# amisr/volumetricinterp

Measured on AMD Instinct MI355X. Metric: fit+eval timesteps/sec, higher is better.
Workload: dtype f64

## Files before the change

### volumetricinterp_amd/csrc/vi_jacobi.hip

```cpp
#include "vi_common.h"
#include "vi_solver.h"

#include <cstdlib>
#include <cstring>

#ifdef VI_STAMPS
__device__ unsigned long long g_jacobi_stamps[16];
#define VI_STAMP(k)                                                                          \
    do {                                                                                     \
        const unsigned long long t_ = __builtin_readcyclecounter();                          \
        if (blockIdx.x == 0 && (threadIdx.x == 0 || threadIdx.x == blockDim.x - 64))         \
            g_jacobi_stamps[(threadIdx.x == 0 ? 0 : 8) + (k)] += t_ - stamp_t;               \
        stamp_t = __builtin_readcyclecounter();                                              \
    } while (0)
#else
#define VI_STAMP(k)
#endif

#ifdef VI_ROTHIST
__device__ unsigned long long g_rot_hist[32][2];
#define VI_ROT_COUNT(sweep, r0, r1, r2, r3)                                                                              \
    atomicAdd(&g_rot_hist[(sweep) < 31 ? (sweep) : 31][0],                                                               \
              (unsigned long long)(((r0).y != 0.0) + ((r1).y != 0.0) + ((r2).y != 0.0) + ((r3).y != 0.0)))
#define VI_ROT_SWEEP(sweep)                                                                                               \
    do { if (threadIdx.x == 0) atomicAdd(&g_rot_hist[(sweep) < 31 ? (sweep) : 31][1], 1ull); } while (0)
#endif

#include "vi_jacobi_device.h"
#include "vi_jacobi_v2_device.h"
#include <cstdlib>
#include <cstring>

namespace {

template <int IT>
__global__ __launch_bounds__(IT == 1 ? 768 : 512) void k_jacobi_solve(
    int N, const double* __restrict__ X, const double* __restrict__ scl, const double* __restrict__ y,
    const int* __restrict__ rec, double rcond, double abs_floor, double* __restrict__ C, int* __restrict__ rank,
    double2* __restrict__ rotlog, int64_t log_stride, int max_sweeps, int* __restrict__ sweeps_out,
    double* __restrict__ lam_out, int lam_raw, int* __restrict__ nround_out, unsigned long long* __restrict__ round_acc,
    double conv_tol)
{
    extern __shared__ __align__(16) unsigned char lds_raw[];
    const int64_t sys = blockIdx.x;
    jacobi_system<IT>(lds_raw, N, X + sys * (int64_t)N * N, scl ? scl[sys] : 1.0, y + (int64_t)(rec ? rec[sys] : sys) * N, rcond,
                      abs_floor, C + sys * N, rank ? rank + sys : nullptr, rotlog + sys * log_stride, max_sweeps,
                      sweeps_out ? sweeps_out + sys : nullptr, lam_out ? lam_out + sys * N : nullptr, lam_raw,
                      nround_out ? nround_out + sys : nullptr, round_acc, conv_tol);
}

__global__ __launch_bounds__(768) void k_jacobi_solve_v2(
    int N, const double* __restrict__ X, const double* __restrict__ scl, const double* __restrict__ y,
    const int* __restrict__ rec, double rcond, double abs_floor, double* __restrict__ C, int* __restrict__ rank,
    double2* __restrict__ rotlog, int64_t log_stride, int max_sweeps, int* __restrict__ sweeps_out,
    double* __restrict__ lam_out, int lam_raw, int* __restrict__ nround_out, unsigned long long* __restrict__ round_acc,
    double conv_tol)
{
    extern __shared__ __align__(16) unsigned char lds_raw[];
    const int64_t sys = blockIdx.x;
    jacobi_system_v2(lds_raw, N, X + sys * (int64_t)N * N, scl ? scl[sys] : 1.0, y + (int64_t)(rec ? rec[sys] : sys) * N, rcond,
                     abs_floor, C + sys * N, rank ? rank + sys : nullptr, rotlog + sys * log_stride, max_sweeps,
                     sweeps_out ? sweeps_out + sys : nullptr, lam_out ? lam_out + sys * N : nullptr, lam_raw,
                     nround_out ? nround_out + sys : nullptr, round_acc, conv_tol);
}

template <int CPW>
__global__ __launch_bounds__(64) void k_jacobi_vectors_wave(int N, const double2* __restrict__ rotlog, int64_t log_stride,
                                                            const int* __restrict__ nround_in, double* __restrict__ Vout)
{
    const int64_t sys = blockIdx.y;
    jacobi_vector_strip<CPW>(N, rotlog + sys * log_stride, nround_in[sys], blockIdx.x * CPW, threadIdx.x,
                             Vout + sys * (int64_t)N * N);
}

}

#ifdef VI_STAMPS
extern "C" int vi_debug_jacobi_stamps(double* out, int reset)
{
    unsigned long long h[16];
    if (hipMemcpyFromSymbol(h, HIP_SYMBOL(g_jacobi_stamps), sizeof(h)) != hipSuccess) return -1;
    for (int i = 0; i < 16; ++i) out[i] = (double)h[i];
    if (reset) {
        memset(h, 0, sizeof(h));
        if (hipMemcpyToSymbol(HIP_SYMBOL(g_jacobi_stamps), h, sizeof(h)) != hipSuccess) return -1;
    }
    return 0;
}
#endif

#ifdef VI_ROTHIST
extern "C" int vi_debug_rot_hist(double* out, int reset)
{
    unsigned long long h[32][2];
    if (hipMemcpyFromSymbol(h, HIP_SYMBOL(g_rot_hist), sizeof(h)) != hipSuccess) return -1;
    for (int i = 0; i < 32; ++i) { out[2 * i] = (double)h[i][0]; out[2 * i + 1] = (double)h[i][1]; }
    if (reset) {
        memset(h, 0, sizeof(h));
        if (hipMemcpyToSymbol(HIP_SYMBOL(g_rot_hist), h, sizeof(h)) != hipSuccess) return -1;
    }
    return 0;
}
#endif

namespace {

int jacobi_nsb(int N)
{
    const int M = ((N + 3) & ~3) / 4;
    return M * (M - 1) / 2;
}
void jacobi_geometry(int N, int& threads, int& it)
{
    const int nsb = jacobi_nsb(N);
    if (nsb <= 768) {
        it = 1;
        threads = ((nsb + 63) / 64) * 64;
        if (threads < 64) threads = 64;
    } else {
        threads = 512;
        it = (nsb + 511) / 512;
    }
}

}

bool vi_jacobi_use_v2(int N)
{
    static const bool v1 = vi_env_is("VINTERP_K3", "v1");
    if (v1) return false;
    int threads, it;
    jacobi_geometry(N, threads, it);
    const int M = ((N + 3) & ~3) / 4;
    static const int minm = [] { const int v = vi_env_int("VINTERP_K3_MINM", 24); return v < 3 ? 3 : v; }();
    return it == 1 && M >= minm && M <= 64 && threads + 64 <= 768;
}

size_t vi_jacobi_lds_bytes(int N)
{
    const int Np = (N + 3) & ~3, M = Np / 4;
    const int nt = Np * (Np + 1) / 2;
    size_t b = (size_t)(nt + 2 * Np) * 8 + (size_t)4 * M * 16 + 16 * 8;
    if (vi_jacobi_use_v2(N)) b += (size_t)4 * M * 16 + (size_t)4 * M * 8 + 16 + (size_t)14 * M * 4;
    return (b + 15) & ~(size_t)15;
}

bool vi_jacobi_supported(int N)
{
    int threads, it;
    jacobi_geometry(N, threads, it);
    return N >= 8 && vi_jacobi_lds_bytes(N) <= 159 * 1024 && it <= 3 && ((N + 3) / 4) <= 64;
}

static int64_t jacobi_log_stride(int N, int max_sweeps)
{
    const int Np = (N + 3) & ~3, m = Np / 2, M = Np / 4;
    return (int64_t)max_sweeps * m * 4 * M;
}
size_t vi_jacobi_log_bytes(int N, int max_sweeps) { return (size_t)jacobi_log_stride(N, max_sweeps) * sizeof(double2); }

template <int IT>
static int launch_jacobi(vi_ctx* c, int threads, int64_t B, int N, const double* d_X, const double* d_scl, const double* d_y,
                         const int* d_rec, double rcond, double* d_C, int* d_rank, void* d_log, int max_sweeps,
                         int* d_sweeps, double* d_lam, int lam_raw, int* d_nround, double abs_floor, int64_t log_stride_in,
                         double conv_tol)
{
    const size_t shm = vi_jacobi_lds_bytes(N);
    VI_HIP(hipFuncSetAttribute((const void*)k_jacobi_solve<IT>, hipFuncAttributeMaxDynamicSharedMemorySize, (int)shm));
    const int64_t log_stride = log_stride_in > 0 ? log_stride_in : jacobi_log_stride(N, max_sweeps);
    const int slot = (int)(c->solve_launches % vi_ctx::NSOLVE_EV);
    if (c->solve_timing) VI_HIP(hipEventRecord(c->evs[slot][0], c->stream));
    hipLaunchKernelGGL(k_jacobi_solve<IT>, dim3((unsigned)B), dim3(threads), shm, c->stream, N, d_X, d_scl, d_y, d_rec,
                       rcond, abs_floor, d_C, d_rank, (double2*)d_log, log_stride, max_sweeps, d_sweeps, d_lam, lam_raw, d_nround,
                       c->solve_timing ? c->d_rounds : nullptr, conv_tol);
    VI_HIP(hipGetLastError());
    if (c->solve_timing) {
        VI_HIP(hipEventRecord(c->evs[slot][1], c->stream));
        c->solve_launches += 1;
        c->solve_systems += B;
    }
    return VI_OK;
}

int vi_jacobi_solve(vi_ctx* c, int64_t B, int N, const double* d_X, const double* d_scl, const double* d_y,
                    const int* d_rec, double rcond, double* d_C, int* d_rank, void* d_log, int max_sweeps,
                    int* d_sweeps, double* d_lam, int lam_raw, int* d_nround, double abs_floor, int64_t log_stride, double conv_tol)
{
    int threads, it;
    jacobi_geometry(N, threads, it);
    if (vi_jacobi_use_v2(N)) {
        const size_t shm = vi_jacobi_lds_bytes(N);
        VI_HIP(hipFuncSetAttribute((const void*)k_jacobi_solve_v2, hipFuncAttributeMaxDynamicSharedMemorySize, (int)shm));
        const int64_t ls = log_stride > 0 ? log_stride : jacobi_log_stride(N, max_sweeps);
        const int slot = (int)(c->solve_launches % vi_ctx::NSOLVE_EV);
        if (c->solve_timing) VI_HIP(hipEventRecord(c->evs[slot][0], c->stream));
        hipLaunchKernelGGL(k_jacobi_solve_v2, dim3((unsigned)B), dim3(threads + 64), shm, c->stream, N, d_X, d_scl, d_y, d_rec, rcond,
                           abs_floor, d_C, d_rank, (double2*)d_log, ls, max_sweeps, d_sweeps, d_lam, lam_raw, d_nround,
                           c->solve_timing ? c->d_rounds : nullptr, conv_tol);
        VI_HIP(hipGetLastError());
        if (c->solve_timing) {
            VI_HIP(hipEventRecord(c->evs[slot][1], c->stream));
            c->solve_launches += 1;
            c->solve_systems += B;
        }
        return VI_OK;
    }
#define VI_J(IT) return launch_jacobi<IT>(c, threads, B, N, d_X, d_scl, d_y, d_rec, rcond, d_C, d_rank, d_log, max_sweeps, d_sweeps, d_lam, lam_raw, d_nround, abs_floor, log_stride, conv_tol)
    if (it <= 1) VI_J(1);
    if (it <= 2) VI_J(2);
    VI_J(3);
#undef VI_J
}

bool vi_jacobi_vectors_supported(int N) { return vi_jacobi_supported(N); }

int vi_jacobi_vectors(vi_ctx* c, int64_t B, int N, const void* d_log, int max_sweeps, const int* d_nround, double* d_V,
                      int64_t log_stride_in)
{
    const int64_t log_stride = log_stride_in > 0 ? log_stride_in : jacobi_log_stride(N, max_sweeps);
    const int64_t cols = B * N, target = (int64_t)8 * c->n_cu;
#define VI_VEC(CPW)                                                                                                           \
    hipLaunchKernelGGL(k_jacobi_vectors_wave<CPW>, dim3((unsigned)((N + CPW - 1) / CPW), (unsigned)B), dim3(64), 0, c->stream, \
                       N, (const double2*)d_log, log_stride, d_nround, d_V)
    if (cols <= target) VI_VEC(1);
    else if (cols <= 2 * target) VI_VEC(2);
    else if (cols <= 4 * target) VI_VEC(4);
    else VI_VEC(8);
#undef VI_VEC
    VI_HIP(hipGetLastError());
    return VI_OK;
}
```

### volumetricinterp_amd/csrc/vi_jacobi_v2_device.h

```cpp
#pragma once
#include "vi_jacobi_device.h"

namespace {

__device__ __forceinline__ void lds_signal(int* w, int n)
{
    asm volatile("s_waitcnt lgkmcnt(0)" ::: "memory");
    __hip_atomic_fetch_add(w, n, __ATOMIC_RELAXED, __HIP_MEMORY_SCOPE_WORKGROUP);
}
template <bool SLEEP = true>
__device__ __forceinline__ void lds_wait(int* w, int target, int& bad)
{
    const int tgt = __builtin_amdgcn_readfirstlane(target);
    int spins = 0;
#pragma nounroll
    for (;;) {
        const int v = __builtin_amdgcn_readfirstlane(__hip_atomic_load(w, __ATOMIC_RELAXED, __HIP_MEMORY_SCOPE_WORKGROUP));
        if (v >= tgt) break;
        if (++spins > (1 << 22)) { bad = 1; break; }
        if (SLEEP) __builtin_amdgcn_s_sleep(1);
    }
    asm volatile("" ::: "memory");
}

__device__ __forceinline__ void jacobi_system_v2(
    unsigned char* lds_raw, int N, const double* __restrict__ Xs, double sc, const double* __restrict__ ys, double rcond,
    double abs_floor, double* __restrict__ Cs, int* __restrict__ rank_s, double2* __restrict__ logp, int max_sweeps,
    int* __restrict__ sweeps_s, double* __restrict__ lam_s, int lam_raw, int* __restrict__ nround_s,
    unsigned long long* __restrict__ round_acc, double conv_tol = 0.0)
{
    const int NT = blockDim.x;
    const int Np = (N + 3) & ~3;
    const int m = Np >> 1;
    const int M = Np >> 2;
    const int nsb = (M * (M - 1)) >> 1;
    const int ntri = 16 * nsb + 10 * M;
    const int dg = 16 * nsb;
    double* A = reinterpret_cast<double*>(lds_raw);
    double* yv = A + ntri;
    double2* cs0 = reinterpret_cast<double2*>(yv + 2 * Np);
    double* nd = reinterpret_cast<double*>(cs0 + 8 * M);
    double* mb = nd + 16;
    int* sync = reinterpret_cast<int*>(mb + 4 * M);
    int* dtab = sync + 4;

    const int tid = threadIdx.x;
    const int nw = NT >> 6;
    const bool setup = tid < 64;

    int ka = 0, kb = 1, ksrc = 0, dst[16];
    bool live = false;
    int serves = -1, q0 = 0;
    {
        int* otab = reinterpret_cast<int*>(A);
        int* wcnt = otab + NT;
        const int lane = tid & 63, wv = tid >> 6;
        const int kn = tid - 64;
        bool isd = false;
        int sv = 0;
        if (!setup && kn < nsb) {
            int bb = (int)((1.0f + sqrtf(1.0f + 8.0f * (float)kn)) * 0.5f);
            while ((bb * (bb - 1)) / 2 > kn) --bb;
            while (((bb + 1) * bb) / 2 <= kn) ++bb;
            const int aa = kn - (bb * (bb - 1)) / 2;
            if (aa == 0 && bb == 1) { isd = true; sv = 0; }
            else if (aa == 0 && bb == 2) { isd = true; sv = 1; }
            else if (aa == M - 2 && bb == M - 1) { isd = true; sv = M - 1; }
            else if (aa >= 1 && bb == aa + 2) { isd = true; sv = aa + 1; }
        }
        const bool plain = !setup && kn < nsb && !isd;
        const unsigned long long mn = __ballot(plain);
        if (lane == 0) wcnt[wv] = __popcll(mn);
        __syncthreads();
        int before = 0;
        for (int w = 0; w < wv; ++w) before += wcnt[w];
        const unsigned long long below = lane ? (~0ull >> (64 - lane)) : 0ull;
        if (isd) otab[sv] = kn;
        if (plain) otab[M + before + __popcll(mn & below)] = kn;
        __syncthreads();
        if (!setup && kn < nsb) ksrc = otab[kn];
        __syncthreads();
    }
    if (!setup) {
        const int ko = tid - 64;
        live = ko < nsb;
        const int k = live ? ksrc : 0;
        int b = (int)((1.0f + sqrtf(1.0f + 8.0f * (float)k)) * 0.5f);
        while ((b * (b - 1)) / 2 > k) --b;
        while (((b + 1) * b) / 2 <= k) ++b;
        const int a = k - (b * (b - 1)) / 2;
        ka = live ? a : 0;
        kb = live ? b : 1;
        ksrc = k;
#pragma unroll
        for (int r = 0; r < 4; ++r)
#pragma unroll
            for (int c = 0; c < 4; ++c) dst[4 * r + c] = tri4(slot_next(4 * ka + r, M), slot_next(4 * kb + c, M), M);
        if (live) {
            if (a == 0 && b == 1) { serves = 0; q0 = 2; }
            else if (a == 0 && b == 2) { serves = 1; q0 = 10; }
            else if (a == M - 2 && b == M - 1) { serves = M - 1; q0 = 0; }
            else if (a >= 1 && b == a + 2) { serves = a + 1; q0 = 2; }
        }
    } else {
#pragma unroll
        for (int e = 0; e < 16; ++e) dst[e] = 0;
        if (tid < M) {
#pragma unroll
            for (int r = 0; r < 4; ++r) {
                dtab[(10 + r) * M + tid] = slot_next(4 * tid + r, M);
#pragma unroll
                for (int c = r; c < 4; ++c) dtab[j10(r, c) * M + tid] = tri4(slot_next(4 * tid + r, M), slot_next(4 * tid + c, M), M);
            }
        }
    }

    double mxd = 0.0;
    for (int e = tid; e < Np * Np; e += NT) {
        const int i = e / Np, j = e - i * Np;
        if (j > i) continue;
        const double v = (i < N && j < N) ? Xs[(int64_t)i * N + j] : 0.0;
        A[tri4(i, j, M)] = v;
        if (i == j) mxd = fmax(mxd, fabs(v));
    }
    for (int s = tid; s < Np; s += NT) yv[s] = s < N ? ys[s] : 0.0;
    for (int o = 32; o > 0; o >>= 1) mxd = fmax(mxd, __shfl_xor(mxd, o));
    if ((tid & 63) == 0) nd[tid >> 6] = mxd;
    if (tid == 0) { sync[0] = 0; sync[1] = 0; sync[2] = 0; }
    __syncthreads();
    mxd = 0.0;
    for (int w = 0; w < nw; ++w) mxd = fmax(mxd, nd[w]);
    const double drop = rcond * mxd;
    const double eps2 = 2.220446049250313e-16 * 2.220446049250313e-16;
    const double conv2 = conv_tol > 0.0 ? conv_tol * conv_tol : VI_CONV_FACTOR * VI_CONV_FACTOR * eps2;
    int sweep = 0, ycur = 0;
    bool converged = false;
    int64_t nround = 0;
    int bad = 0;
    int tgt_mb = 0, tgt_st = 0;
#ifdef VI_STAMPS
    unsigned long long stamp_t = __builtin_readcyclecounter();
#endif
    if (setup) {
        double d[4][4], yy[4];
        bool in_regs = false;
        int dd[10], yd[4];
#pragma unroll
        for (int j = 0; j < 10; ++j) dd[j] = tid < M ? dtab[j * M + tid] : 0;
#pragma unroll
        for (int p = 0; p < 4; ++p) yd[p] = tid < M ? dtab[(10 + p) * M + tid] : 0;
        for (; sweep < max_sweeps; ++sweep) {
            int rotated = 0;
            for (int r = 0; r < m; ++r, ++nround) {
                const bool intra = r == 0;
                double2* cs = cs0 + (nround & 1) * (4 * M);
                if (tid < M) {
                    if (!in_regs) {
#pragma unroll
                        for (int p = 0; p < 4; ++p)
#pragma unroll
                            for (int q = p; q < 4; ++q) d[p][q] = d[q][p] = A[dg + j10(p, q) * M + tid];
#pragma unroll
                        for (int p = 0; p < 4; ++p) yy[p] = yv[ycur * Np + 4 * tid + p];
                    }
                    double2 r0, r1, r2 = make_double2(1.0, 0.0), r3 = make_double2(1.0, 0.0);
                    if (intra) {
                        rot_stage<0, 1, 2, 3>(d, yy, drop, abs_floor, rotated, r0, r1);
                    } else {
                        rot_stage<0, 2, 1, 3>(d, yy, drop, abs_floor, rotated, r0, r1);
                        rot_stage<0, 3, 1, 2>(d, yy, drop, abs_floor, rotated, r2, r3);
                    }
                    cs[tid] = r0;
                    cs[M + tid] = r1;
                    cs[2 * M + tid] = r2;
                    cs[3 * M + tid] = r3;
                    double2* lp = logp + nround * (int64_t)(4 * M) + tid;
                    lp[0] = r0;
                    lp[M] = r1;
                    lp[2 * M] = r2;
                    lp[3 * M] = r3;
                }
                VI_STAMP(0);
                __syncthreads();
                VI_STAMP(1);
                if (tid < M) {
                    if (r == m - 1) {
#pragma unroll
                        for (int p = 0; p < 4; ++p) {
                            yv[(ycur ^ 1) * Np + yd[p]] = yy[p];
#pragma unroll
                            for (int q = p; q < 4; ++q) A[dd[j10(p, q)]] = d[p][q];
                        }
                    } else if (!intra) {
                        A[dd[j10(0, 2)]] = d[0][2];
                        A[dd[j10(0, 3)]] = d[0][3];
                        A[dd[j10(1, 2)]] = d[1][2];
                        A[dd[j10(1, 3)]] = d[1][3];
                    }
                }
                VI_STAMP(2);
                if (!intra) {
                    const int last = M - 1;
                    const double pu00 = WaveReplay::from_prev(d[0][0]), pu01 = WaveReplay::from_prev(d[0][1]), pu11 = WaveReplay::from_prev(d[1][1]);
                    const double pv00 = WaveReplay::from_prev(d[2][2]), pv01 = WaveReplay::from_prev(d[2][3]), pv11 = WaveReplay::from_prev(d[3][3]);
                    const double nv00 = WaveReplay::from_next(d[2][2]), nv01 = WaveReplay::from_next(d[2][3]), nv11 = WaveReplay::from_next(d[3][3]);
                    const double pyu0 = WaveReplay::from_prev(yy[0]), pyu1 = WaveReplay::from_prev(yy[1]);
                    const double pyv0 = WaveReplay::from_prev(yy[2]), pyv1 = WaveReplay::from_prev(yy[3]);
                    const double nyv0 = WaveReplay::from_next(yy[2]), nyv1 = WaveReplay::from_next(yy[3]);
                    const double o00 = d[0][0], o01 = d[0][1], o11 = d[1][1], oy0 = yy[0], oy1 = yy[1];
                    const bool l0 = tid == 0, l1 = tid == 1, ll = tid == last;
                    d[0][0] = l0 ? o00 : (l1 ? pv00 : pu00);
                    d[0][1] = d[1][0] = l0 ? o01 : (l1 ? pv01 : pu01);
                    d[1][1] = l0 ? o11 : (l1 ? pv11 : pu11);
                    d[2][2] = ll ? o00 : nv00;
                    d[2][3] = d[3][2] = ll ? o01 : nv01;
                    d[3][3] = ll ? o11 : nv11;
                    yy[0] = l0 ? oy0 : (l1 ? pyv0 : pyu0);
                    yy[1] = l0 ? oy1 : (l1 ? pyv1 : pyu1);
                    yy[2] = ll ? oy0 : nyv0;
                    yy[3] = ll ? oy1 : nyv1;
                    VI_STAMP(3);
                    lds_wait<false>(sync, tgt_mb + M, bad);
                    if (tid < M) {
                        d[0][2] = d[2][0] = mb[tid];
                        d[0][3] = d[3][0] = mb[M + tid];
                        d[1][2] = d[2][1] = mb[2 * M + tid];
                        d[1][3] = d[3][1] = mb[3 * M + tid];
                    }
                }
                in_regs = true;
                VI_STAMP(4);
                if (tid == 0) lds_signal(sync + 2, 1);
                if (!intra) tgt_mb += M;
                tgt_st += nw;
                ycur ^= 1;
                VI_STAMP(7);
            }
            if (!__syncthreads_or(rotated)) { ++sweep; converged = true; break; }
            int viol = 0;
            if (tid < M) {
#pragma unroll
                for (int p = 0; p < 4; ++p)
#pragma unroll
                    for (int q = p + 1; q < 4; ++q)
                        viol |= would_rotate(A[dg + p * M + tid], A[dg + q * M + tid], A[dg + j10(p, q) * M + tid], drop,
                                             abs_floor, conv2);
            }
            if (!__syncthreads_or(viol)) { ++sweep; converged = true; break; }
        }
    } else {
        for (; sweep < max_sweeps; ++sweep) {
            for (int r = 0; r < m; ++r, ++nround) {
                const bool intra = r == 0;
                const double2* csc = cs0 + (nround & 1) * (4 * M);
                double b[16];
                lds_wait(sync + 2, tgt_st, bad);
                if (live) {
#pragma unroll
                    for (int e = 0; e < 16; ++e) b[e] = A[ksrc + e * nsb];
                }
                VI_STAMP(0);
                asm volatile("s_barrier" ::: "memory");
                VI_STAMP(1);
                if (tid < 128 && !intra) __builtin_amdgcn_s_setprio(3);
                if (live) {
                    const double2 ra0 = csc[ka], ra1 = csc[M + ka];
                    const double2 rb0 = csc[kb], rb1 = csc[M + kb];
                    if (intra) {
                        rot_rows<0, 1>(b, ra0);
                        rot_rows<2, 3>(b, ra1);
                        rot_cols<0, 1>(b, rb0);
                        rot_cols<2, 3>(b, rb1);
#pragma unroll
                        for (int e = 0; e < 16; ++e) A[ksrc + e * nsb] = b[e];
                    } else {
                        const double2 ra2 = csc[2 * M + ka], ra3 = csc[3 * M + ka];
                        const double2 rb2 = csc[2 * M + kb], rb3 = csc[3 * M + kb];
                        rot_rows<0, 2>(b, ra0);
                        rot_rows<1, 3>(b, ra1);
                        rot_rows<0, 3>(b, ra2);
                        rot_rows<1, 2>(b, ra3);
                        rot_cols<0, 2>(b, rb0);
                        rot_cols<1, 3>(b, rb1);
                        rot_cols<0, 3>(b, rb2);
                        rot_cols<1, 2>(b, rb3);
                        if (serves >= 0) {
                            const bool qa = q0 == 2, qb = q0 == 10;
                            mb[serves] = qa ? b[2] : (qb ? b[10] : b[0]);
                            mb[M + serves] = qa ? b[3] : (qb ? b[11] : b[1]);
                            mb[2 * M + serves] = qa ? b[6] : (qb ? b[14] : b[4]);
                            mb[3 * M + serves] = qa ? b[7] : (qb ? b[15] : b[5]);
                            lds_signal(sync, 1);
                        }
                    }
                }
                VI_STAMP(2);
                if (!intra) {
                    if (tid < 128) __builtin_amdgcn_s_setprio(0);
                    if (live) {
#pragma unroll
                        for (int e = 0; e < 16; ++e) A[dst[e]] = b[e];
                    }
                }
                VI_STAMP(4);
                if ((tid & 63) == 0) lds_signal(sync + 2, 1);
                tgt_st += nw;
                ycur ^= 1;
                VI_STAMP(7);
            }
            if (!__syncthreads_or(0)) { ++sweep; converged = true; break; }
            int viol = 0;
            if (live) {
#pragma unroll
                for (int r = 0; r < 4; ++r) {
                    const double app = A[dg + r * M + ka];
#pragma unroll
                    for (int c = 0; c < 4; ++c)
                        viol |= would_rotate(app, A[dg + c * M + kb], A[ksrc + (4 * r + c) * nsb], drop, abs_floor, conv2);
                }
            }
            if (!__syncthreads_or(viol)) { ++sweep; converged = true; break; }
        }
    }
    if (__syncthreads_or(bad)) converged = false;
    double* yc = yv + ycur * Np;
    double mx = 0.0;
    for (int i = tid; i < Np; i += NT) mx = fmax(mx, fabs(A[dg + (i & 3) * M + (i >> 2)]));
    for (int o = 32; o > 0; o >>= 1) mx = fmax(mx, __shfl_xor(mx, o));
    if ((tid & 63) == 0) nd[tid >> 6] = mx;
    __syncthreads();
    mx = 0.0;
    for (int w = 0; w < nw; ++w) mx = fmax(mx, nd[w]);
    const double thr = rcond * mx;
    int rk = 0;
    for (int i = tid; i < Np; i += NT) {
        const double lam = A[dg + (i & 3) * M + (i >> 2)];
        const bool keep = fabs(lam) > thr;
        yc[i] = keep ? yc[i] / (lam * sc) : 0.0;
        rk += keep ? 1 : 0;
        if (lam_s && i < N) lam_s[i] = lam_raw ? lam : lam * sc;
    }
    __syncthreads();
    for (int o = 32; o > 0; o >>= 1) rk += __shfl_xor(rk, o);
    if ((tid & 63) == 0) nd[tid >> 6] = (double)rk;
    __syncthreads();
    if (tid == 0) {
        double tot = 0.0;
        for (int w = 0; w < nw; ++w) tot += nd[w];
        if (rank_s) *rank_s = (int)tot;
        if (sweeps_s) *sweeps_s = converged ? sweep : max_sweeps + 1;
        if (nround_s) *nround_s = (int)nround;
        if (round_acc) atomicAdd(round_acc, (unsigned long long)nround);
    }
    if (tid < 64) {
        constexpr int PF = 4;
        WaveReplay W;
        W.init(tid, M);
        W.load(yc, M);
        const bool has = tid < M;
        for (int64_t r1 = nround; r1 > 0; r1 -= PF) {
            const int nb = r1 >= PF ? PF : (int)r1;
            double2 pf[PF][4];
#pragma unroll
            for (int u = 0; u < PF; ++u) {
#pragma unroll
                for (int j = 0; j < 4; ++j) pf[u][j] = make_double2(1.0, 0.0);
                if (u < nb && has) {
                    const double2* lp = logp + (r1 - 1 - u) * (int64_t)(4 * M) + tid;
#pragma unroll
                    for (int j = 0; j < 4; ++j) pf[u][j] = lp[j * M];
                }
            }
#pragma unroll
            for (int u = 0; u < PF; ++u)
                if (u < nb) W.round(pf[u], ((r1 - 1 - u) % m) == 0);
        }
        W.store(yc, M);
    }
    __syncthreads();
    for (int s = tid; s < N; s += NT) Cs[s] = yc[s];
}

}
```

Before: 3552.

## Split v2 Jacobi solver into phases, software-pipeline rotation replay and vectorize matrix load

Splits the v2 Jacobi solver into setup, load, iterate, truncate and replay phases and adds optional per-phase cycle counters. The replay of logged rotations now keeps a rolling prefetch window of depth 8 in registers, issuing loads for later rounds while applying earlier ones to hide global-memory latency. The matrix load now reads rows per wave as aligned double2 pairs with unrolling instead of a per-element divide/modulo loop. The cost is more register pressure in the replay wave and a more complex load path.

New measurement: 3668, median of 6. +3.3%, better.

```diff
diff --git a/volumetricinterp_amd/csrc/vi_jacobi.hip b/volumetricinterp_amd/csrc/vi_jacobi.hip
--- a/volumetricinterp_amd/csrc/vi_jacobi.hip
+++ b/volumetricinterp_amd/csrc/vi_jacobi.hip
@@ -13,6 +13,15 @@
             g_jacobi_stamps[(threadIdx.x == 0 ? 0 : 8) + (k)] += t_ - stamp_t;               \
         stamp_t = __builtin_readcyclecounter();                                              \
     } while (0)
+__device__ unsigned long long g_jacobi_phases[16];
+#define VI_PHASE(k)                                                                                          \
+    do {                                                                                                     \
+        const unsigned long long t_ = __builtin_readcyclecounter();                                          \
+        if (threadIdx.x == 0) atomicAdd(&g_jacobi_phases[(conv_tol > 0.0 ? 0 : 8) + (k)], t_ - phase_t);     \
+        phase_t = __builtin_readcyclecounter();                                                              \
+    } while (0)
+#define VI_PHASE_COUNT()                                                                                     \
+    do { if (threadIdx.x == 0) atomicAdd(&g_jacobi_phases[(conv_tol > 0.0 ? 0 : 8) + 7], 1ull); } while (0)
 #else
 #define VI_STAMP(k)
 #endif
@@ -58,10 +67,11 @@
 {
     extern __shared__ __align__(16) unsigned char lds_raw[];
     const int64_t sys = blockIdx.x;
-    jacobi_system_v2(lds_raw, N, X + sys * (int64_t)N * N, scl ? scl[sys] : 1.0, y + (int64_t)(rec ? rec[sys] : sys) * N, rcond,
-                     abs_floor, C + sys * N, rank ? rank + sys : nullptr, rotlog + sys * log_stride, max_sweeps,
-                     sweeps_out ? sweeps_out + sys : nullptr, lam_out ? lam_out + sys * N : nullptr, lam_raw,
-                     nround_out ? nround_out + sys : nullptr, round_acc, conv_tol);
+    jacobi_system_v2<V2_REPLAY_AHEAD>(lds_raw, N, X + sys * (int64_t)N * N, scl ? scl[sys] : 1.0,
+                                      y + (int64_t)(rec ? rec[sys] : sys) * N, rcond, abs_floor, C + sys * N,
+                                      rank ? rank + sys : nullptr, rotlog + sys * log_stride, max_sweeps,
+                                      sweeps_out ? sweeps_out + sys : nullptr, lam_out ? lam_out + sys * N : nullptr, lam_raw,
+                                      nround_out ? nround_out + sys : nullptr, round_acc, conv_tol);
 }
 
 template <int CPW>
@@ -84,6 +94,20 @@
     if (reset) {
         memset(h, 0, sizeof(h));
         if (hipMemcpyToSymbol(HIP_SYMBOL(g_jacobi_stamps), h, sizeof(h)) != hipSuccess) return -1;
+    }
+    return 0;
+}
+#endif
+
+#ifdef VI_STAMPS
+extern "C" int vi_debug_jacobi_phases(double* out, int reset)
+{
+    unsigned long long h[16];
+    if (hipMemcpyFromSymbol(h, HIP_SYMBOL(g_jacobi_phases), sizeof(h)) != hipSuccess) return -1;
+    for (int i = 0; i < 16; ++i) out[i] = (double)h[i];
+    if (reset) {
+        memset(h, 0, sizeof(h));
+        if (hipMemcpyToSymbol(HIP_SYMBOL(g_jacobi_phases), h, sizeof(h)) != hipSuccess) return -1;
     }
     return 0;
 }
diff --git a/volumetricinterp_amd/csrc/vi_jacobi_v2_device.h b/volumetricinterp_amd/csrc/vi_jacobi_v2_device.h
--- a/volumetricinterp_amd/csrc/vi_jacobi_v2_device.h
+++ b/volumetricinterp_amd/csrc/vi_jacobi_v2_device.h
@@ -23,36 +23,61 @@
     asm volatile("" ::: "memory");
 }
 
-__device__ __forceinline__ void jacobi_system_v2(
-    unsigned char* lds_raw, int N, const double* __restrict__ Xs, double sc, const double* __restrict__ ys, double rcond,
-    double abs_floor, double* __restrict__ Cs, int* __restrict__ rank_s, double2* __restrict__ logp, int max_sweeps,
-    int* __restrict__ sweeps_s, double* __restrict__ lam_s, int lam_raw, int* __restrict__ nround_s,
-    unsigned long long* __restrict__ round_acc, double conv_tol = 0.0)
-{
-    const int NT = blockDim.x;
-    const int Np = (N + 3) & ~3;
-    const int m = Np >> 1;
-    const int M = Np >> 2;
-    const int nsb = (M * (M - 1)) >> 1;
-    const int ntri = 16 * nsb + 10 * M;
-    const int dg = 16 * nsb;
-    double* A = reinterpret_cast<double*>(lds_raw);
-    double* yv = A + ntri;
-    double2* cs0 = reinterpret_cast<double2*>(yv + 2 * Np);
-    double* nd = reinterpret_cast<double*>(cs0 + 8 * M);
-    double* mb = nd + 16;
-    int* sync = reinterpret_cast<int*>(mb + 4 * M);
-    int* dtab = sync + 4;
-
-    const int tid = threadIdx.x;
-    const int nw = NT >> 6;
+
+struct V2Frame {
+    int N, NT, Np, m, M, nsb, ntri, dg, tid, nw;
+    double* A;
+    double* yv;
+    double2* cs0;
+    double* nd;
+    double* mb;
+    int* sync;
+    int* dtab;
+    __device__ __forceinline__ V2Frame(unsigned char* lds_raw, int N_)
+    {
+        N = N_;
+        NT = blockDim.x;
+        Np = (N + 3) & ~3;
+        m = Np >> 1;
+        M = Np >> 2;
+        nsb = (M * (M - 1)) >> 1;
+        ntri = 16 * nsb + 10 * M;
+        dg = 16 * nsb;
+        A = reinterpret_cast<double*>(lds_raw);
+        yv = A + ntri;
+        cs0 = reinterpret_cast<double2*>(yv + 2 * Np);
+        nd = reinterpret_cast<double*>(cs0 + 8 * M);
+        mb = nd + 16;
+        sync = reinterpret_cast<int*>(mb + 4 * M);
+        dtab = sync + 4;
+        tid = threadIdx.x;
+        nw = NT >> 6;
+    }
+};
+
+struct V2Geo {
+    int ka, kb, ksrc, dst[16];
+    bool live;
+    int serves, q0;
+};
+
+struct V2Run {
+    int sweep, ycur;
+    bool converged;
+    int64_t nround;
+};
+
+__device__ __forceinline__ void v2_setup(const V2Frame& f, V2Geo& g)
+{
+    const int NT = f.NT, M = f.M, nsb = f.nsb, tid = f.tid;
+    int* dtab = f.dtab;
     const bool setup = tid < 64;
 
     int ka = 0, kb = 1, ksrc = 0, dst[16];
     bool live = false;
     int serves = -1, q0 = 0;
     {
-        int* otab = reinterpret_cast<int*>(A);
+        int* otab = reinterpret_cast<int*>(f.A);
         int* wcnt = otab + NT;
         const int lane = tid & 63, wv = tid >> 6;
         const int kn = tid - 64;
@@ -114,26 +139,96 @@
             }
         }
     }
-
+    g.ka = ka;
+    g.kb = kb;
+    g.ksrc = ksrc;
+#pragma unroll
+    for (int e = 0; e < 16; ++e) g.dst[e] = dst[e];
+    g.live = live;
+    g.serves = serves;
+    g.q0 = q0;
+}
+
+__device__ __forceinline__ double v2_load_rows(const V2Frame& f, const double* __restrict__ Xs, const double* __restrict__ ys,
+                                               double* yd, int w, int nwl, int tl, int ntl)
+{
+    constexpr int UR = 4;
+    const int N = f.N, Np = f.Np, M = f.M, nsb = f.nsb, dg = f.dg, lane = f.tid & 63;
+    double* A = f.A;
     double mxd = 0.0;
-    for (int e = tid; e < Np * Np; e += NT) {
-        const int i = e / Np, j = e - i * Np;
-        if (j > i) continue;
-        const double v = (i < N && j < N) ? Xs[(int64_t)i * N + j] : 0.0;
-        A[tri4(i, j, M)] = v;
-        if (i == j) mxd = fmax(mxd, fabs(v));
-    }
-    for (int s = tid; s < Np; s += NT) yv[s] = s < N ? ys[s] : 0.0;
+    for (int i0 = w; i0 < Np; i0 += UR * nwl) {
+        double2 v[UR][2];
+#pragma unroll
+        for (int u = 0; u < UR; ++u) {
+            const int i = i0 + u * nwl;
+            const double* row = Xs + (int64_t)i * N;
+            const bool al = (reinterpret_cast<uintptr_t>(row) & 15) == 0;
+#pragma unroll
+            for (int p = 0; p < 2; ++p) {
+                const int j = 2 * lane + 128 * p;
+                v[u][p] = make_double2(0.0, 0.0);
+                if (i < N && j <= i) {
+                    if (al && j < i) {
+                        v[u][p] = *reinterpret_cast<const double2*>(row + j);
+                    } else {
+                        v[u][p].x = row[j];
+                        if (j < i) v[u][p].y = row[j + 1];
+                    }
+                }
+            }
+        }
+#pragma unroll
+        for (int u = 0; u < UR; ++u) {
+            const int i = i0 + u * nwl;
+            const int a = i >> 2, r = i & 3, base = (a * (a - 1)) >> 1;
+#pragma unroll
+            for (int p = 0; p < 2; ++p) {
+                const int j = 2 * lane + 128 * p;
+                if (i < Np && j <= i) {
+                    const int b = j >> 2, c = j & 3;
+                    const int s0 = b == a ? dg + j10(c, r) * M + a : (4 * c + r) * nsb + base + b;
+                    const int s1 = b == a ? dg + j10(c + 1, r) * M + a : s0 + 4 * nsb;
+                    A[s0] = v[u][p].x;
+                    if (j < i) A[s1] = v[u][p].y;
+                    if (j == i) mxd = fmax(mxd, fabs(v[u][p].x));
+                    if (j + 1 == i) mxd = fmax(mxd, fabs(v[u][p].y));
+                }
+            }
+        }
+    }
+    for (int s = tl; s < Np; s += ntl) yd[s] = s < N ? ys[s] : 0.0;
+    return mxd;
+}
+
+__device__ __forceinline__ double v2_load_close(const V2Frame& f, double mxd)
+{
+    const int tid = f.tid;
     for (int o = 32; o > 0; o >>= 1) mxd = fmax(mxd, __shfl_xor(mxd, o));
-    if ((tid & 63) == 0) nd[tid >> 6] = mxd;
-    if (tid == 0) { sync[0] = 0; sync[1] = 0; sync[2] = 0; }
+    if ((tid & 63) == 0) f.nd[tid >> 6] = mxd;
+    if (tid == 0) { f.sync[0] = 0; f.sync[1] = 0; f.sync[2] = 0; }
     __syncthreads();
     mxd = 0.0;
-    for (int w = 0; w < nw; ++w) mxd = fmax(mxd, nd[w]);
-    const double drop = rcond * mxd;
-    const double eps2 = 2.220446049250313e-16 * 2.220446049250313e-16;
-    const double conv2 = conv_tol > 0.0 ? conv_tol * conv_tol : VI_CONV_FACTOR * VI_CONV_FACTOR * eps2;
-    int sweep = 0, ycur = 0;
+    for (int w = 0; w < f.nw; ++w) mxd = fmax(mxd, f.nd[w]);
+    return mxd;
+}
+
+__device__ __forceinline__ void v2_iterate(const V2Frame& f, const V2Geo& g, double drop, double abs_floor, double conv2,
+                                           int max_sweeps, double2* __restrict__ logp, V2Run& run)
+{
+    const int Np = f.Np, m = f.m, M = f.M, nsb = f.nsb, dg = f.dg, tid = f.tid, nw = f.nw;
+    double* A = f.A;
+    double* yv = f.yv;
+    double2* cs0 = f.cs0;
+    double* mb = f.mb;
+    int* sync = f.sync;
+    const int* dtab = f.dtab;
+    const bool setup = tid < 64;
+    const int ka = g.ka, kb = g.kb, ksrc = g.ksrc, serves = g.serves, q0 = g.q0;
+    const bool live = g.live;
+    int dst[16];
+#pragma unroll
+    for (int e = 0; e < 16; ++e) dst[e] = g.dst[e];
+    int sweep = 0, ycur = run.ycur;
     bool converged = false;
     int64_t nround = 0;
     int bad = 0;
@@ -323,7 +418,23 @@
         }
     }
     if (__syncthreads_or(bad)) converged = false;
-    double* yc = yv + ycur * Np;
+    run.sweep = sweep;
+    run.ycur = ycur;
+    run.converged = converged;
+    run.nround = nround;
+}
+
+__device__ __forceinline__ void v2_truncate(const V2Frame& f, const V2Run& run, double sc, double rcond, int* __restrict__ rank_s,
+                                            int max_sweeps, int* __restrict__ sweeps_s, double* __restrict__ lam_s, int lam_raw,
+                                            int* __restrict__ nround_s, unsigned long long* __restrict__ round_acc)
+{
+    const int N = f.N, NT = f.NT, Np = f.Np, M = f.M, dg = f.dg, tid = f.tid, nw = f.nw;
+    const double* A = f.A;
+    double* nd = f.nd;
+    const int sweep = run.sweep;
+    const bool converged = run.converged;
+    const int64_t nround = run.nround;
+    double* yc = f.yv + run.ycur * Np;
     double mx = 0.0;
     for (int i = tid; i < Np; i += NT) mx = fmax(mx, fabs(A[dg + (i & 3) * M + (i >> 2)]));
     for (int o = 32; o > 0; o >>= 1) mx = fmax(mx, __shfl_xor(mx, o));
@@ -352,9 +463,16 @@
         if (nround_s) *nround_s = (int)nround;
         if (round_acc) atomicAdd(round_acc, (unsigned long long)nround);
     }
-    if (tid < 64) {
+}
+
+__device__ __forceinline__ WaveReplay v2_replay(const V2Frame& f, const V2Run& run, const double2* __restrict__ logp)
+{
+    const int m = f.m, M = f.M, tid = f.tid;
+    const int64_t nround = run.nround;
+    const double* yc = f.yv + run.ycur * f.Np;
+    WaveReplay W;
+    {
         constexpr int PF = 4;
-        WaveReplay W;
         W.init(tid, M);
         W.load(yc, M);
         const bool has = tid < M;
@@ -375,10 +493,93 @@
             for (int u = 0; u < PF; ++u)
                 if (u < nb) W.round(pf[u], ((r1 - 1 - u) % m) == 0);
         }
-        W.store(yc, M);
-    }
+    }
+    return W;
+}
+
+template <int DEPTH>
+__device__ __forceinline__ WaveReplay v2_replay_ahead(const V2Frame& f, const V2Run& run, const double2* __restrict__ logp)
+{
+    const int m = f.m, M = f.M, tid = f.tid;
+    const int nround = (int)run.nround;
+    const double* yc = f.yv + run.ycur * f.Np;
+    WaveReplay W;
+    W.init(tid, M);
+    W.load(yc, M);
+    const bool has = tid < M;
+    const double2* lbase = logp + (has ? tid : 0);
+    double2 pf[DEPTH][4];
+    auto issue = [&](double2 (&p)[4], int rr) {
+        const double2* lp = lbase + (rr > 0 ? rr : 0) * (int64_t)(4 * M);
+#pragma unroll
+        for (int j = 0; j < 4; ++j) p[j] = lp[j * M];
+    };
+    int rm = nround > 0 ? (nround - 1) % m : 0;
+    auto apply = [&](const double2 (&p)[4]) {
+        double2 q[4];
+#pragma unroll
+        for (int j = 0; j < 4; ++j) q[j] = has ? p[j] : make_double2(1.0, 0.0);
+        W.round(q, rm == 0);
+        rm = rm == 0 ? m - 1 : rm - 1;
+    };
+#pragma unroll
+    for (int u = 0; u < DEPTH; ++u) issue(pf[u], nround - 1 - u);
+    int r1 = nround;
+    for (; r1 >= DEPTH; r1 -= DEPTH) {
+#pragma unroll
+        for (int u = 0; u < DEPTH; ++u) {
+            apply(pf[u]);
+            issue(pf[u], r1 - 1 - u - DEPTH);
+        }
+    }
+#pragma unroll
+    for (int u = 0; u < DEPTH; ++u)
+        if (u < r1) apply(pf[u]);
+    return W;
+}
+
+#ifndef VI_PHASE
+#define VI_PHASE(k)
+#define VI_PHASE_COUNT()
+#endif
+
+template <int AHEAD = 0>
+__device__ __forceinline__ void jacobi_system_v2(
+    unsigned char* lds_raw, int N, const double* __restrict__ Xs, double sc, const double* __restrict__ ys, double rcond,
+    double abs_floor, double* __restrict__ Cs, int* __restrict__ rank_s, double2* __restrict__ logp, int max_sweeps,
+    int* __restrict__ sweeps_s, double* __restrict__ lam_s, int lam_raw, int* __restrict__ nround_s,
+    unsigned long long* __restrict__ round_acc, double conv_tol = 0.0)
+{
+    const V2Frame f(lds_raw, N);
+    V2Geo g;
+#ifdef VI_STAMPS
+    unsigned long long phase_t = __builtin_readcyclecounter();
+#endif
+    v2_setup(f, g);
+    VI_PHASE(0);
+    const double mxd = v2_load_close(f, v2_load_rows(f, Xs, ys, f.yv, f.tid >> 6, f.nw, f.tid, f.NT));
+    VI_PHASE(1);
+    const double drop = rcond * mxd;
+    const double eps2 = 2.220446049250313e-16 * 2.220446049250313e-16;
+    const double conv2 = conv_tol > 0.0 ? conv_tol * conv_tol : VI_CONV_FACTOR * VI_CONV_FACTOR * eps2;
+    V2Run run;
+    run.ycur = 0;
+    v2_iterate(f, g, drop, abs_floor, conv2, max_sweeps, logp, run);
+    VI_PHASE(2);
+    v2_truncate(f, run, sc, rcond, rank_s, max_sweeps, sweeps_s, lam_s, lam_raw, nround_s, round_acc);
+    VI_PHASE(3);
+    double* yc = f.yv + run.ycur * f.Np;
+    if (f.tid < 64) {
+        if (AHEAD > 0) v2_replay_ahead<(AHEAD > 0 ? AHEAD : 1)>(f, run, logp).store(yc, f.M);
+        else v2_replay(f, run, logp).store(yc, f.M);
+    }
+    VI_PHASE(4);
     __syncthreads();
-    for (int s = tid; s < N; s += NT) Cs[s] = yc[s];
-}
-
-}
+    for (int s = f.tid; s < N; s += f.NT) Cs[s] = yc[s];
+    VI_PHASE(5);
+    VI_PHASE_COUNT();
+}
+
+constexpr int V2_REPLAY_AHEAD = 8;
+
+}
```
